# PixelClear/OclPathTracer

Measured on AMD Instinct MI355X. Metric: Msamples/sec (pixels x spp / s), cornellbox.bin 1024x1024, higher is better.
Workload: dtype f32; 1 GPU; BASELINE configs[2]: cornellbox.bin 1024x1024, 256 spp, depth 16, full path; render_lanes=2, checkpointed_launches=True, staging_ring_bytes=402653184, workspace_bytes=477453648

## Files before the change

### oclpathtracer_amd/csrc/pt_kernels.h

```cpp
#pragma once

#include <hip/hip_runtime.h>
#include <stdint.h>

struct PtRawTriangle { float p1[4], p2[4], p3[4]; int32_t id; char pad[12]; };
struct PtRawMaterial { float albedo[4], emissive[4]; float roughness; int32_t type; char pad[24]; };
static_assert(sizeof(PtRawTriangle) == 64 && sizeof(PtRawMaterial) == 64, "record layout");

struct PtPrepTriangle {
    float p1[3];
    float e1[3];
    float e2[3];
    float pad0[3];
    float n[3];
    int32_t id;
};
static_assert(sizeof(PtPrepTriangle) == 64, "prep layout");

struct PtBvhNode {
    float lmin[3]; uint32_t link_l;
    float lmax[3]; uint32_t link_r;
    float rmin[3]; uint32_t pad0;
    float rmax[3]; uint32_t pad1;
};
// ... 24 lines not shown
#define PT_LDS_TRI_STRIDE 12
#define PT_LDS_TRI_MAX 256

struct PtCamera {
    float eye[3], view[3], hol[3], up[3];
    float angle;
};

struct PtTraceParams {
    const PtPrepTriangle* tris;
    const PtRawMaterial* mats;
    float* rad;
    float* rad1;
    unsigned int* batch_counter;
    unsigned long long* stats;
    int32_t width, height;
    float inv_width, inv_height, aspect;
    int32_t frame_begin;
    int32_t frame_count;
    uint32_t chunk_f0;
    uint32_t slot_frames;
    uint32_t ring_phase;
    uint32_t ring_magic;
    uint32_t rad1_off;
    int32_t max_bounces, ntri, nmat;
    int32_t stripe_rows, n_ranks, rank;
    uint32_t npix_local;
    uint32_t batches_per_frame, total_batches;
    uint32_t batch;
    float quad_delta1;
    float ray_radius;
    const float* p1tab;
    float p1_lo, p1_hi;
    const PtBvh8Node* bvh;
    int32_t bvh_records;
    PtBvhGrid grid;
    const PtPrepTriangle* bigtab;
    const int32_t* bigidx;
    int32_t nbig;
    const uint2* pmask;
    unsigned int* bvh_flags;
    int32_t bvh_stack_limit;
    uint32_t* carry;
    uint32_t carry_in_waves;
    uint32_t carry_out;
    PtCamera cam;
};
#define PT_QUEUE_SHARDS 8
#define PT_QUEUE_SHARD_WORDS 1056
#define PT_QUEUE_STOP_WORD (PT_QUEUE_SHARDS * PT_QUEUE_SHARD_WORDS)
#define PT_QUEUE_WORDS ((PT_QUEUE_SHARDS + 1) * PT_QUEUE_SHARD_WORDS)
#define PT_CARRY_RECORDS 64
#define PT_CARRY_STRIDE_DW (16 + PT_CARRY_RECORDS * 15)

struct PtFoldParams {
    const float* rad;
    float4* fb;
    uint32_t npix_local;
    int32_t frame_begin, frame_count;
    unsigned int* reset_counter;
    unsigned int* reset_counter2;
};

#define PT_PREP_WORDS 12
__host__ __device__ static inline unsigned ptk_order_key(float f)
{
    unsigned u;
    __builtin_memcpy(&u, &f, sizeof u);
    return (u & 0x80000000u) ? ~u : (u | 0x80000000u);
}
__host__ __device__ static inline float ptk_order_float(unsigned k)
{
    const unsigned u = (k & 0x80000000u) ? (k & 0x7fffffffu) : ~k;
    float f;
    __builtin_memcpy(&f, &u, sizeof f);
    return f;
}
hipError_t ptk_prep_triangles(const PtRawTriangle* raw, PtPrepTriangle* out, int ntri, unsigned int* det_bound_bits,
                              hipStream_t s);
hipError_t ptk_prep_quad_margins(PtPrepTriangle* out, int ntri, float diameter, float delta1, float* p1tab, const float anchor[3], hipStream_t s);
#define PT_P1_STRIDE 24
static inline size_t ptk_p1tab_floats(int ntri) { return (size_t)((ntri / 2 + 1) / 2) * PT_P1_STRIDE; }
hipError_t ptk_primary_masks(const PtTraceParams& p, hipStream_t s);
struct PtSearchMode {
    bool bvh;
    bool det_bounded;
    int quads;
};
hipError_t ptk_trace(const PtTraceParams& p, int num_blocks, PtSearchMode m, bool tally, bool wide, hipStream_t s);
#define PT_BVH_NEAR_EYE 4.0f
hipError_t ptk_bvh_big_raw(const PtRawTriangle* raw, const int* bigidx, int nbig, PtRawTriangle* out, hipStream_t s);
static inline size_t ptk_bvh_record_count(int ntri) { return 2 * (size_t)(ntri > 0 ? ntri : 0); }
size_t ptk_bvh_temp_bytes(int ntri);
#define PT_BVH_BIG_MAX 64
#define PT_BVH_RAY_EPS 1.2e-4f
hipError_t ptk_bvh_build(const PtRawTriangle* raw, const PtPrepTriangle* prep, int ntri, PtBvh8Node* recs,
                         PtPrepTriangle* bigtab, int* bigidx, int* nbig_dev, PtBvhGrid* grid_dev, unsigned* used_dev, void* temp, size_t temp_bytes,
                         hipStream_t s);
#define PT_DET_BOUND_MAX 2.0e19f
#define PT_BVH_AUTO_MIN 512
hipError_t ptk_fold(const PtFoldParams& p, hipStream_t s);
hipError_t ptk_assemble_stripes(const float4* gathered, float4* image, int width, int height, int stripe_rows,
                                int n_ranks, int slab_rows, hipStream_t s);
hipError_t ptk_tonemap_ppm(const float4* fb, int32_t* rgb, size_t npix, hipStream_t s);
hipError_t ptk_fill_i32(int32_t* dst, int32_t value, int n, hipStream_t s);
hipError_t ptk_math(const float* in, float* out, int n, hipStream_t s);
// ... 139 lines not shown
```

### oclpathtracer_amd/csrc/pt_kernels.hip

```cpp
#include "pt_kernels.h"

#include "pt_device_math.h"

#include <type_traits>

typedef const __attribute__((address_space(4))) float* pt_const_f32p;

PTK_DEV unsigned pt_lane_id() { return __builtin_amdgcn_mbcnt_hi(~0u, __builtin_amdgcn_mbcnt_lo(~0u, 0u)); }
PTK_DEV unsigned pt_mbcnt(unsigned long long m) { return __builtin_amdgcn_mbcnt_hi((unsigned)(m >> 32), __builtin_amdgcn_mbcnt_lo((unsigned)m, 0u)); }

typedef const __attribute__((address_space(4))) PtTraceParams* pt_kargs_p;
PTK_DEV pt_kargs_p pt_kargs()
{
    pt_kargs_p k = (pt_kargs_p)__builtin_amdgcn_kernarg_segment_ptr();
    asm volatile("" : "+s"(k));
    return k;
}
PTK_DEV f3 pt_anchor()
{
    const pt_kargs_p K = pt_kargs();
    return mk3(K->cam.eye[0], K->cam.eye[1], K->cam.eye[2]);
}
#define PT_ARG(field) (LATE ? K->field : P.field)

// ... 625 lines not shown
            for (int jj = 0; jj < n; ++jj) {
                const PtTriRec r = pt_load_tri(T, base + jj);
                float pvx = pt_fma(d.y, r.e2z, -(d.z * r.e2y));
                float pvy = pt_fma(d.z, r.e2x, -(d.x * r.e2z));
                float pvz = pt_fma(d.x, r.e2y, -(d.y * r.e2x));
                float det = pt_fma(r.e1z, pvz, pt_fma(r.e1y, pvy, r.e1x * pvx));
                bool keep = !(det < 1e-8f || -det > 1e-8f);
                float inv_det = 1.0f / det;
                float tvx = o.x - r.p1x, tvy = o.y - r.p1y, tvz = o.z - r.p1z;
                float u = pt_fma(tvz, pvz, pt_fma(tvy, pvy, tvx * pvx)) * inv_det;
                keep = keep && !(u < 0.0f || u > 1.0f);
                float qvx = pt_fma(tvy, r.e1z, -(tvz * r.e1y));
                float qvy = pt_fma(tvz, r.e1x, -(tvx * r.e1z));
                float qvz = pt_fma(tvx, r.e1y, -(tvy * r.e1x));
                float v = pt_fma(d.z, qvz, pt_fma(d.y, qvy, d.x * qvx)) * inv_det;
                keep = keep && !(v < 0.0f || u + v > 1.0f);
                float tt = pt_fma(r.e2z, qvz, pt_fma(r.e2y, qvy, r.e2x * qvx)) * inv_det;
                keep = keep && (tt > 0.0f && tt < 1e20f);
                mx |= (keep ? 1u : 0u) << (n - 1 - jj);
            }
            atomicAdd(&vstat[0], (unsigned long long)n);
            atomicAdd(&vstat[1], (unsigned long long)__popc(mx));
            atomicAdd(&vstat[2], (unsigned long long)__popc(m));
            atomicAdd(&vstat[3], (unsigned long long)__popc(mx & ~m));
        }
#endif
        if (!alive) m = 0u;
        pt_pass2_chunk<DET_BOUNDED, LDS_TABLE>(m, base, n, tris, o, d, tmax, hu, hv, hidx, tl, lane, steps);
    }
    pt_pass2_finish<DET_BOUNDED, LDS_TABLE>(tris, o, d, tmax, hu, hv, hidx, tl, lane, steps);
    return steps;
}


struct PtPath {
    f3 o, d;
    f3 mask, L;
    uint32_t seed;
    int bounce;
    unsigned ro;
    unsigned fl;
};

PTK_DEV unsigned pt_ring_offset(unsigned lp, unsigned frame)
{
    const pt_kargs_p KR = pt_kargs();
    const unsigned fr = frame + KR->ring_phase, S = KR->slot_frames;
    const unsigned r = fr - __umulhi(fr, KR->ring_magic) * (2u * S);
    const bool upper = r >= S;
    return (upper ? KR->rad1_off : 0u) + ((upper ? r - S : r) * KR->npix_local + lp) * 12u;
}


template <bool DET_BOUNDED, bool LATE>
PTK_DEV bool pt_shade_path(const PtTraceParams& P, PtPath& s, float tmax, float hu, float hv, int hidx)
{
    const pt_kargs_p K = pt_kargs();
    bool finished = false;
    if (hidx < 0) {
        const float bg = pt_max(0.45f, 0.0f);
        s.L = add3(s.L, scale3(s.mask, bg));
        finished = true;
    } else {
        float phi = PTK_TWO_PI * pt_random_float(s.seed);
        float xi = pt_random_float(s.seed);
        float sp, cp;
        __builtin_amdgcn_sched_barrier(0);
        pt_sincos(phi, sp, cp);
        __builtin_amdgcn_sched_barrier(0);

        const float4 nid = *reinterpret_cast<const float4*>(reinterpret_cast<const char*>(PT_ARG(tris)) + (size_t)((unsigned)hidx * 64u) + 48);
        const f3 N = mk3(nid.x, nid.y, nid.z);
        const int nm1 = PT_ARG(nmat) - 1;
        int mid = __float_as_int(nid.w);
        mid = mid < 0 ? 0 : mid;
        mid = mid > nm1 ? nm1 : mid;
        f3 p = add3(s.o, scale3(s.d, tmax));
        float w = 1.0f - hu - hv;
        f3 n = normalize3(add3(add3(scale3(N, hu), scale3(N, hv)), scale3(N, w)));

        const PtRawMaterial* mat = reinterpret_cast<const PtRawMaterial*>(reinterpret_cast<const char*>(PT_ARG(mats)) + (size_t)((unsigned)mid * 64u));
        const float4 alb = *reinterpret_cast<const float4*>(mat->albedo);
        const float4 emi = *reinterpret_cast<const float4*>(mat->emissive);
        const float rough = mat->roughness;
        const int type = mat->type;

        s.L.x = s.L.x + s.mask.x * emi.x * 3.0f;
        s.L.y = s.L.y + s.mask.y * emi.y * 3.0f;
        s.L.z = s.L.z + s.mask.z * emi.z * 3.0f;

        n = dot3(n, s.d) < 0.0f ? n : scale3(n, -1.0f);
        f3 wo = neg3(s.d);

        f3 axis = __builtin_fabsf(n.x) > 0.001f ? mk3(0.0f, 1.0f, 0.0f) : mk3(1.0f, 0.0f, 0.0f);
        f3 tv = normalize3(cross3(axis, n));
        f3 sv = cross3(n, tv);
        float cos_arg = 1.0f - xi;
#if PT_GGX_FAST
        if (type == 2) cos_arg = pt_div_by(cos_arg, xi * (rough * rough - 1.0f) + 1.0f);
#else
        if (type == 2) cos_arg = cos_arg / (xi * (rough * rough - 1.0f) + 1.0f);
#endif
        const float cosTheta = pt_sqrt(cos_arg);
        const float sin_arg = type == 2 ? pt_max(0.0f, 1.0f - cosTheta * cosTheta) : xi;
        const float sinTheta = pt_sqrt(sin_arg);
        f3 a = scale3(scale3(sv, cp), sinTheta);
        f3 b = scale3(scale3(tv, sp), sinTheta);
        f3 c = scale3(n, cosTheta);
        f3 sdir = normalize3_unit(add3(add3(a, b), c));

        f3 wi = sdir;
        f3 color = mk3(0.0f, 0.0f, 0.0f);
        float pdf = 0.0f;
        float dwin = 0.0f;
        if (type == 1) {
            dwin = dot3(wi, n);
            pdf = dwin * PTK_INV_PI;
            color = mk3(alb.x * PTK_INV_PI, alb.y * PTK_INV_PI, alb.z * PTK_INV_PI);
        } else if (type == 2) {
            float k2 = 2.0f * dot3(wo, sdir);
            wi = add3(neg3(wo), scale3(sdir, k2));
            dwin = dot3(wi, n);
            float dwon = dot3(wo, n);
            if (!(dwin * dwon < 0.0f)) {
                float r2 = rough * rough;
                const float gd = cosTheta * cosTheta * (r2 - 1.0f) + 1.0f;
#if PT_GGX_FAST
                const float D = pt_div(r2 * PTK_INV_PI, gd * gd);
                float g;
                pt_div_pair(D * cosTheta, 4.0f * dot3(wo, sdir), D, 4.0f * dwin * dwon, pdf, g);
#else
                float D = r2 * PTK_INV_PI / (gd * gd);
                pdf = D * cosTheta / (4.0f * dot3(wo, sdir));
                float g = D / (4.0f * dwin * dwon);
#endif
                color = mk3(alb.x * g * 2.0f, alb.y * g * 2.0f, alb.z * g * 2.0f);
            }
        }
        if (pdf <= 0.0f) {
            finished = true;
        } else {
            float qx = color.x * dwin, qy = color.y * dwin, qz = color.z * dwin;
            pt_div3(qx, qy, qz, pdf);
            s.mask.x = s.mask.x * qx;
            s.mask.y = s.mask.y * qy;
            s.mask.z = s.mask.z * qz;
            s.bounce++;
            if (s.bounce >= PT_ARG(max_bounces)) {
                finished = true;
            } else {
                s.o = add3(p, scale3(wi, 0.01f));
                s.d = normalize3_unit(wi);
            }
        }
    }
    if (finished) {
        const pt_kargs_p KR = pt_kargs();
        float* const rad = KR->rad;
        const unsigned rad1_off = KR->rad1_off;
        typedef float pt_f3v __attribute__((ext_vector_type(3), aligned(4)));
        pt_f3v v;
        v.x = pt_max(s.L.x, 0.0f);
        v.y = pt_max(s.L.y, 0.0f);
        v.z = pt_max(s.L.z, 0.0f);
        if (rad1_off != 0u) {
            *reinterpret_cast<pt_f3v*>(reinterpret_cast<char*>(rad) + (size_t)s.ro) = v;
        } else {
            const unsigned fr = s.fl + KR->ring_phase, S = KR->slot_frames;
            const unsigned r = fr - __umulhi(fr, KR->ring_magic) * (2u * S);
            float* out = (r < S ? rad : KR->rad1) + ((size_t)(r < S ? r : r - S) * KR->npix_local + s.ro) * 3u;
            *reinterpret_cast<pt_f3v*>(out) = v;
        }
    }
    return finished;
}

template <bool DET_BOUNDED, bool LATE>
PTK_DEV void pt_shade(const PtTraceParams& P, PtPath& s, bool& alive, float tmax, float hu, float hv, int hidx)
{
    if (pt_shade_path<DET_BOUNDED, LATE>(P, s, tmax, hu, hv, hidx)) alive = false;
}

PTK_DEV void pt_flush_counters(const PtTraceParams& P, unsigned lane, unsigned n_rays, unsigned n_samples)
{
    if (!P.stats) return;
    const unsigned long long r = n_rays, s = n_samples;
    if (lane == 0) {
        atomicAdd(&P.stats[0], s);
        atomicAdd(&P.stats[1], r);
    }
}

#define PT_POOL 64

struct PtWaveQueue {
    unsigned pix, end, frame;
    unsigned row, col;
    unsigned sl, within;
    unsigned g;
};

#define PT_Q_EMPTY 0xffffffffu

template <bool LATE>
PTK_DEV void pt_queue_locate(const PtTraceParams& P, pt_kargs_p K, PtWaveQueue& q)
{
    q.row = q.pix / (unsigned)PT_ARG(width);
    q.col = q.pix - q.row * (unsigned)PT_ARG(width);
    q.sl = q.row / (unsigned)PT_ARG(stripe_rows);
    q.within = q.row - q.sl * (unsigned)PT_ARG(stripe_rows);
}

template <bool LATE>
PTK_DEV bool pt_queue_refill(const PtTraceParams& P, unsigned lane, PtWaveQueue& q, unsigned empty_mask)
{
    const pt_kargs_p K = pt_kargs();
    if (q.pix != q.end) return true;
    if (q.g == PT_Q_EMPTY) return false;
    const unsigned total = PT_ARG(total_batches);
    unsigned sh = q.g, b = 0u;
    bool got = false;
    for (unsigned tries = 0u; tries < PT_QUEUE_SHARDS && total != 0u; ++tries, sh = (sh + 1u) & (PT_QUEUE_SHARDS - 1u)) {
        if ((empty_mask >> sh) & 1u) continue;
        unsigned k = 0u;
        if (lane == 0) k = atomicAdd(PT_ARG(batch_counter) + sh * PT_QUEUE_SHARD_WORDS, 1u);
        k = __builtin_amdgcn_readfirstlane(k);
        b = k * PT_QUEUE_SHARDS + sh;
        if (b < total) { got = true; break; }
        unsigned seen = 0u;
        if (lane == 0u) seen = atomicOr(PT_ARG(batch_counter) + PT_QUEUE_STOP_WORD, 1u << sh);
        empty_mask |= (1u << sh) | (unsigned)__builtin_amdgcn_readfirstlane(seen);
    }
    if (!got) { q.g = PT_Q_EMPTY; return false; }
    q.g = sh;
    const unsigned f = b / PT_ARG(batches_per_frame);
    const unsigned bi = b - f * PT_ARG(batches_per_frame);
    q.frame = PT_ARG(chunk_f0) + f;
    q.pix = bi * PT_ARG(batch);
    const unsigned e = q.pix + PT_ARG(batch);
    q.end = e < PT_ARG(npix_local) ? e : PT_ARG(npix_local);
    pt_queue_locate<LATE>(P, K, q);
    return true;
}

struct PtPathSlots {
    float4* A;
    unsigned* W;
    unsigned fs, ws, wk;
    PTK_DEV float4& vec(unsigned j, unsigned k) const { return A[j * fs + k]; }
    PTK_DEV unsigned& word(unsigned j, unsigned k) const { return W[j * ws + wk * k]; }
};

#define PT_POOL_DWORDS (PT_POOL * 15)
PTK_DEV PtPathSlots pt_pool_slots(float4* pool) { return { pool, reinterpret_cast<unsigned*>(pool + 3 * PT_POOL), PT_POOL, 1u, 3u }; }
PTK_DEV PtPathSlots pt_carry_slots(uint32_t* region) { return { (float4*)(region + 16), region + 16 + PT_CARRY_RECORDS * 12, PT_CARRY_RECORDS, PT_CARRY_RECORDS, 1u }; }

PTK_DEV void pt_path_store(const PtPathSlots& S, unsigned k, const PtPath& s)
{
    S.vec(0, k) = make_float4(s.o.x, s.o.y, s.o.z, s.d.x);
    S.vec(1, k) = make_float4(s.d.y, s.d.z, s.mask.x, s.mask.y);
    S.vec(2, k) = make_float4(s.mask.z, s.L.x, s.L.y, s.L.z);
    S.word(0, k) = s.seed;
    S.word(1, k) = s.ro;
    S.word(2, k) = s.fl | ((unsigned)s.bounce << 16);
}

PTK_DEV void pt_path_load(const PtPathSlots& S, unsigned k, PtPath& s)
{
    const float4 a0 = S.vec(0, k), a1 = S.vec(1, k), a2 = S.vec(2, k);
    const unsigned w2 = S.word(2, k);
    s.o = mk3(a0.x, a0.y, a0.z);
    s.d = mk3(a0.w, a1.x, a1.y);
    s.mask = mk3(a1.z, a1.w, a2.x);
    s.L = mk3(a2.y, a2.z, a2.w);
    s.seed = S.word(0, k);
    s.ro = S.word(1, k);
    s.fl = w2 & 0xffffu;
    s.bounce = (int)(w2 >> 16);
}

PTK_DEV void pt_pool_push(float4* pool, unsigned& pool_n, const PtPath& s, pt_lanes& alive)
{
    const pt_lanes live = alive;
    if (PT_ON(live)) {
        const unsigned k = pool_n + pt_mbcnt(live);
        pt_path_store(pt_pool_slots(pool), k, s);
    }
    pool_n += (unsigned)__popcll(live);
    alive = 0ull;
}

PTK_DEV void pt_pool_pop(float4* pool, unsigned& pool_n, PtPath& s, pt_lanes& alive)
{
    const pt_lanes need = ~alive;
    const unsigned n_need = (unsigned)__popcll(need);
    const unsigned take = n_need < pool_n ? n_need : pool_n;
    if (take == 0u) return;
    __builtin_amdgcn_fence(__ATOMIC_RELEASE, "wavefront");
    __builtin_amdgcn_wave_barrier();
    __builtin_amdgcn_fence(__ATOMIC_ACQUIRE, "wavefront");
    const unsigned rank = pt_mbcnt(need);
    const pt_lanes taking = need & PT_LANES(rank < take);
    if (PT_ON(taking)) {
        const unsigned k = pool_n - 1u - rank;
        pt_path_load(pt_pool_slots(pool), k, s);
    }
    alive |= taking;
    pool_n -= take;
    __builtin_amdgcn_fence(__ATOMIC_RELEASE, "wavefront");
    __builtin_amdgcn_wave_barrier();
    __builtin_amdgcn_fence(__ATOMIC_ACQUIRE, "wavefront");
}


PTK_DEV void pt_carry_header(uint32_t* region, unsigned n, const PtWaveQueue& q, unsigned n_rays, unsigned n_samples, unsigned n_carried)
{
    region[0] = n;
    region[1] = q.pix;
    region[2] = q.end;
    region[3] = q.frame;
    region[4] = n_rays;
    region[5] = n_samples;
    region[6] = n_carried + n + (q.end - q.pix);
}

PTK_DEV void pt_carry_store(uint32_t* region, unsigned lane, float4* pool, unsigned pool_n, const PtWaveQueue& q, unsigned n_rays, unsigned n_samples,
                            unsigned n_carried)
{
    __builtin_amdgcn_fence(__ATOMIC_RELEASE, "wavefront");
    __builtin_amdgcn_wave_barrier();
    __builtin_amdgcn_fence(__ATOMIC_ACQUIRE, "wavefront");
    if (lane < pool_n) {
        const PtPathSlots from = pt_pool_slots(pool), to = pt_carry_slots(region);
        for (unsigned j = 0; j < 3u; ++j) to.vec(j, lane) = from.vec(j, lane);
        for (unsigned j = 0; j < 3u; ++j) to.word(j, lane) = from.word(j, lane);
    }
    if (lane == 0u) pt_carry_header(region, pool_n, q, n_rays, n_samples, n_carried);
}

PTK_DEV void pt_carry_store_lanes(uint32_t* region, unsigned lane, const PtPath& s, bool alive, const PtWaveQueue& q, unsigned n_rays, unsigned n_samples,
                                  unsigned n_carried)
{
    const unsigned long long live = __ballot(alive);
    const unsigned n_live = (unsigned)__popcll(live);
    if (alive) {
        const unsigned k = pt_mbcnt(live);
        pt_path_store(pt_carry_slots(region), k, s);
    }
    if (lane == 0u) pt_carry_header(region, n_live, q, n_rays, n_samples, n_carried);
}

template <bool LATE>
PTK_DEV void pt_carry_load(const PtTraceParams& P, uint32_t* region, unsigned lane, PtPath& s, bool& alive, PtWaveQueue& q, unsigned& n_rays,
                           unsigned& n_samples, unsigned& n_carried)
{
    const pt_kargs_p K = pt_kargs();
    const unsigned n = __builtin_amdgcn_readfirstlane(region[0]);
    n_rays = __builtin_amdgcn_readfirstlane(region[4]);
    n_samples = __builtin_amdgcn_readfirstlane(region[5]);
    n_carried = __builtin_amdgcn_readfirstlane(region[6]);
    q.pix = __builtin_amdgcn_readfirstlane(region[1]);
    q.end = __builtin_amdgcn_readfirstlane(region[2]);
    q.frame = __builtin_amdgcn_readfirstlane(region[3]);
    pt_queue_locate<LATE>(P, K, q);
    if (lane < n) {
        pt_path_load(pt_carry_slots(region), lane, s);
        alive = true;
    }
}

template <bool LATE>
PTK_DEV int pt_queue_next(const PtTraceParams& P, unsigned lane, PtWaveQueue& q, const PtPath& s, pt_lanes alive)
{
    const pt_kargs_p K = pt_kargs();
    unsigned empty_mask = 0u;
    if (PT_ARG(carry_out) != 0u) {
        if (lane == 0u) empty_mask = __hip_atomic_load(PT_ARG(batch_counter) + PT_QUEUE_STOP_WORD, __ATOMIC_RELAXED, __HIP_MEMORY_SCOPE_AGENT);
        empty_mask = (unsigned)__builtin_amdgcn_readfirstlane(empty_mask);
        if (empty_mask == (1u << PT_QUEUE_SHARDS) - 1u && !(q.pix != q.end && q.frame < PT_ARG(chunk_f0)) && (alive & PT_LANES(s.fl < PT_ARG(chunk_f0))) == 0ull)
            return 2;
    }
    return pt_queue_refill<LATE>(P, lane, q, empty_mask) ? 1 : 0;
}

template <bool LATE>
PTK_DEV unsigned pt_stripe_row(const PtTraceParams& P, pt_kargs_p K, unsigned sl, unsigned within)
{
    return (sl * (unsigned)PT_ARG(n_ranks) + (unsigned)PT_ARG(rank)) * (unsigned)PT_ARG(stripe_rows) + within;
}

template <bool LATE>
PTK_DEV void pt_pixel_xy(const PtTraceParams& P, pt_kargs_p K, unsigned lp, unsigned& x, unsigned& grow)
{
    const unsigned lr = lp / (unsigned)PT_ARG(width);
    x = lp - lr * (unsigned)PT_ARG(width);
    grow = lr;
    if (PT_ARG(n_ranks) > 1) {
        const unsigned sl = lr / (unsigned)PT_ARG(stripe_rows);
        grow = pt_stripe_row<LATE>(P, K, sl, lr - sl * (unsigned)PT_ARG(stripe_rows));
    }
}

template <bool LATE>
PTK_DEV void pt_sample_begin(const PtTraceParams& P, pt_kargs_p K, unsigned x, unsigned grow, unsigned lp, unsigned frame, PtPath& s)
{
    const unsigned gid = grow * (unsigned)PT_ARG(width) + x;
    const int f = PT_ARG(frame_begin) - (int)PT_ARG(chunk_f0) + (int)frame;
    s.seed = gid + pt_hash_u32((uint32_t)f);
    pt_generate_ray((int)x, (int)grow, PT_ARG(inv_width), PT_ARG(inv_height), PT_ARG(aspect), PT_CAM_K(K->cam), s.seed, s.o, s.d);
    s.mask = mk3(1.0f, 1.0f, 1.0f);
    s.L = mk3(0.0f, 0.0f, 0.0f);
    s.bounce = 0;
    s.ro = K->rad1_off != 0u ? pt_ring_offset(lp, frame) : lp;
    s.fl = frame;
}

template <bool LATE>
PTK_DEV bool pt_start_fresh(const PtTraceParams& P, unsigned lane, PtWaveQueue& q, PtPath& s, pt_lanes& alive, unsigned& pix0)
{
    const pt_kargs_p K = pt_kargs();
    pix0 = q.pix;
    const unsigned avail = q.end - q.pix;
    const unsigned count = avail < 64u ? avail : 64u;
    const unsigned W = (unsigned)PT_ARG(width), SR = (unsigned)PT_ARG(stripe_rows);
    if (lane < count) {
        unsigned x = q.col + lane, up = 0u;
        while (x >= W) { x -= W; ++up; }
        unsigned grow = q.row + up;
        if (PT_ARG(n_ranks) > 1) {
            unsigned sl = q.sl, within = q.within + up;
            while (within >= SR) { within -= SR; ++sl; }
            grow = pt_stripe_row<LATE>(P, K, sl, within);
        }
        pt_sample_begin<LATE>(P, K, x, grow, q.pix + lane, q.frame, s);
    }
    alive = count == 64u ? ~0ull : (1ull << count) - 1ull;
    q.pix += count;
    q.col += count;
    while (q.col >= W) {
        q.col -= W;
        ++q.row;
        if (++q.within == SR) { q.within = 0u; ++q.sl; }
    }
    return count == 64u;
}

PTK_DEV PtPath pt_path_idle()
{
    PtPath s;
    s.o = mk3(0.0f, 0.0f, 0.0f); s.d = mk3(0.0f, 0.0f, 1.0f);
    s.mask = mk3(1.0f, 1.0f, 1.0f); s.L = mk3(0.0f, 0.0f, 0.0f);
    s.seed = 0; s.bounce = 0; s.ro = 0; s.fl = 0;
    return s;
}

PTK_DEV unsigned pt_wave_in_wg() { return (unsigned)__builtin_amdgcn_readfirstlane(threadIdx.x >> 6); }
PTK_DEV unsigned pt_wave() { return blockIdx.x * (PT_TRACE_THREADS / 64) + pt_wave_in_wg(); }
PTK_DEV uint32_t* pt_carry_region(uint32_t* carry, unsigned wave) { return carry + (size_t)wave * PT_CARRY_STRIDE_DW; }

PTK_DEV PtTail pt_tail_init(pt_lds_u32* w, unsigned tile, unsigned lane)
{
    PtTail tl;
    tl.keys = (pt_lds_u64*)w;
    tl.list = w + 128;
    tl.wr = tl.rd = 0u;
    tl.kbest = ~0ull; tl.ku = tl.kv = 0.0f;
    tl.tile = tile;
    tl.keys[lane] = ~0ull;
    return tl;
}

PTK_DEV void pt_lds_table_load(const PtPrepTriangle* tris, int n)
{
    const float* g = reinterpret_cast<const float*>(tris);
    for (int k = (int)threadIdx.x; k < n * PT_LDS_TRI_STRIDE; k += PT_TRACE_THREADS) {
        const int tri = k / PT_LDS_TRI_STRIDE, w = k - tri * PT_LDS_TRI_STRIDE;
        pt_lds_tab[k] = g[tri * 16 + w];
    }
}

#define PT_LDS_TILE_DW (32u * PT_LDS_TRI_STRIDE)
template <int LDS_TABLE> __host__ __device__ __forceinline__ unsigned pt_lds_tail_dw() { return 128u + (LDS_TABLE == 1 ? PT_TAIL_LIST / 2u : PT_TAIL_LIST); }
template <int LDS_TABLE> __host__ __device__ __forceinline__ unsigned pt_lds_pools(int ntri) { return LDS_TABLE == 1 ? ntri * PT_LDS_TRI_STRIDE : 0; }
template <int LDS_TABLE, bool POOLS = true> __host__ __device__ __forceinline__ unsigned pt_lds_tails(int ntri) { return pt_lds_pools<LDS_TABLE>(ntri) + (POOLS ? (PT_TRACE_THREADS / 64) * PT_POOL_DWORDS : 0u); }
template <int LDS_TABLE, bool POOLS = true> __host__ __device__ __forceinline__ unsigned pt_lds_tiles(int ntri) { return pt_lds_tails<LDS_TABLE, POOLS>(ntri) + (PT_TRACE_THREADS / 64) * pt_lds_tail_dw<LDS_TABLE>(); }
template <int LDS_TABLE, bool POOLS = true> __host__ __device__ __forceinline__ unsigned pt_lds_total(int ntri) { return pt_lds_tiles<LDS_TABLE, POOLS>(ntri) + (LDS_TABLE == 2 ? (PT_TRACE_THREADS / 64) * PT_LDS_TILE_DW : 0u); }

#ifndef PT_TRACE_UNIT_DIR
#define PT_TRACE_UNIT_DIR 1
#endif
template <bool DET_BOUNDED, int LDS_TABLE, int QUADS>
PTK_DEV void pt_trace_body(const PtTraceParams& P)
{
    const unsigned lane = pt_lane_id();
    pt_const_f32p T = (pt_const_f32p)(const float*)P.tris;
    const int ntri = P.ntri;
    if (LDS_TABLE == 1) {
        pt_lds_table_load(P.tris, ntri);
        __syncthreads();
    }
    const unsigned wave_in_wg = pt_wave_in_wg();
    float4* pool = reinterpret_cast<float4*>(pt_lds_tab + pt_lds_pools<LDS_TABLE>(ntri) + wave_in_wg * PT_POOL_DWORDS);
    unsigned pool_n = 0u;
    PtTail tl = pt_tail_init((pt_lds_u32*)pt_lds_tab + pt_lds_tails<LDS_TABLE>(ntri) + (threadIdx.x >> 6) * pt_lds_tail_dw<LDS_TABLE>(),
                             pt_lds_tiles<LDS_TABLE>(ntri) + (threadIdx.x >> 6) * PT_LDS_TILE_DW, lane);

    PtWaveQueue q = { 0u, 0u, 0u, 0u, 0u, 0u, 0u, 0u };
    pt_lanes alive = 0ull;
    PtPath s = pt_path_idle();
    unsigned n_rays = 0, n_samples = 0, n_carried = 0;
    const unsigned wave = pt_wave();
    if (wave < P.carry_in_waves) {
        bool resumed = false;
        pt_carry_load<true>(P, pt_carry_region(P.carry, wave), lane, s, resumed, q, n_rays, n_samples, n_carried);
        alive = PT_LANES(resumed);
    }
    q.g = wave & (PT_QUEUE_SHARDS - 1u);
#if PT_STAMPS
    unsigned long long t0 = 0, t1 = 0, t2 = 0, t3 = 0, c_regen = 0, c_loop = 0, c_shade = 0, c_iters = 0, c_steps = 0, c_p1 = 0;
#endif

    for (;;) {
        PT_STAMP(t0);
        bool primary = false;
        unsigned pix0 = 0u;
        if (~alive != 0ull) {
            if (pool_n == 0u) {
                const int next = pt_queue_next<true>(P, lane, q, s, alive);
                if (next != 0) {
                    pt_pool_push(pool, pool_n, s, alive);
                    if (next == 2) break;
                    primary = pt_start_fresh<true>(P, lane, q, s, alive, pix0);
                }
            }
            pt_pool_pop(pool, pool_n, s, alive);
        }
        if (alive == 0ull) break;
        PT_STAMP(t1);

        float tmax = 1e20f, hu = 0.0f, hv = 0.0f;
        int hidx = -1;
        unsigned p2steps = 0;
        if (QUADS == 3 && DET_BOUNDED && primary && P.pmask != nullptr)
            p2steps = pt_intersect_primary<DET_BOUNDED, LDS_TABLE>(T, P.tris, ntri, s.o, s.d, PT_ON(alive), tmax, hu, hv, hidx, P.pmask[pix0 + lane], tl, lane,
                                                                   PT_VALIDATE_FILTER && P.stats ? P.stats + 2 : nullptr);
        else
            p2steps = pt_intersect_two_pass<DET_BOUNDED, LDS_TABLE, QUADS, PT_TRACE_UNIT_DIR != 0>(T, P.tris, ntri, s.o, s.d, PT_ON(alive), tmax, hu, hv, hidx,
                                                                                          P.quad_delta1, P.ray_radius,
                                                                                          (pt_const_f32p)P.p1tab, P.p1_lo, P.p1_hi, pt_anchor(), tl, lane,
                                                                                          PT_VALIDATE_FILTER && P.stats ? P.stats + 2 : nullptr,
#if PT_STAMPS
                                                                                          &c_p1
#else
                                                                                          nullptr
#endif
                                                                                          );
#if PT_STAMPS
        c_steps += p2steps;
#else
        (void)p2steps;
#endif

        PT_STAMP(t2);
        n_rays += (unsigned)__popcll(alive);
        bool finished = false;
        if (PT_ON(alive)) finished = pt_shade_path<DET_BOUNDED, true>(P, s, tmax, hu, hv, hidx);
        const pt_lanes done = PT_LANES(finished);
        n_samples += (unsigned)__popcll(done);
        alive &= ~done;
#if PT_STAMPS
        PT_STAMP(t3);
        c_regen += t1 - t0; c_loop += t2 - t1; c_shade += t3 - t2; c_iters++;
#endif
    }

#if PT_STAMPS
    if (P.stats && lane == 0) {
        atomicAdd(&P.stats[2], c_regen);
        atomicAdd(&P.stats[3], c_loop);
        atomicAdd(&P.stats[4], c_shade);
        atomicAdd(&P.stats[5], c_iters);
        atomicAdd(&P.stats[7], c_steps);
        atomicAdd(&P.stats[6], c_p1);
    }
#endif
    {
        const pt_kargs_p K = pt_kargs();
        if (K->carry_out != 0u) {
            pt_carry_store(pt_carry_region(K->carry, wave), lane, pool, pool_n, q, n_rays, n_samples, n_carried);
            return;
        }
    }
#if !PT_STAMPS && !PT_VALIDATE_FILTER
    if (P.stats && lane == 0 && n_carried != 0u) atomicAdd(&P.stats[7], (unsigned long long)n_carried);
#endif
    pt_flush_counters(P, lane, n_rays, n_samples);
}

#ifndef PT_TRACE_WAVES
#define PT_TRACE_WAVES 8
#endif
template <bool DET_BOUNDED, int LDS_TABLE, int QUADS>
__global__ __launch_bounds__(PT_TRACE_THREADS) __attribute__((amdgpu_waves_per_eu(PT_TRACE_WAVES, PT_TRACE_WAVES)))
void pt_trace_kernel(const PtTraceParams P)
{
    pt_trace_body<DET_BOUNDED, LDS_TABLE, QUADS>(P);
}

template <bool DET_BOUNDED>
__global__ __launch_bounds__(PT_TRACE_THREADS) __attribute__((amdgpu_waves_per_eu(6, 6)))
void pt_trace_tiled_kernel(const PtTraceParams P)
{
    pt_trace_body<DET_BOUNDED, 2, 0>(P);
}

#ifndef PT_BVH_STACK
#define PT_BVH_STACK 64
#endif
#ifndef PT_BVH_LDS_STACK
#define PT_BVH_LDS_STACK 8
#endif
#ifndef PT_BVH_REFILL
#define PT_BVH_REFILL 40
#endif

#define PT_BVH_TAIL_DW (128u + PT_TAIL_LIST)
__host__ __device__ __forceinline__ unsigned pt_bvh_lds_stacks() { return PT_BVH_BIG_MAX * PT_LDS_TRI_STRIDE; }
__host__ __device__ __forceinline__ unsigned pt_bvh_lds_tails() { return pt_bvh_lds_stacks() + 2 * PT_BVH_LDS_STACK * PT_TRACE_THREADS; }
__host__ __device__ __forceinline__ unsigned pt_bvh_lds_nxt() { return pt_bvh_lds_tails() + (PT_TRACE_THREADS / 64) * PT_BVH_TAIL_DW; }
__host__ __device__ __forceinline__ unsigned pt_bvh_lds_total() { return pt_bvh_lds_nxt() + 2048u / 4u; }

template <bool LATE>
PTK_DEV void pt_regenerate_lanes(const PtTraceParams& P, unsigned lane, PtWaveQueue& q, PtPath& s, bool& alive)
{
    const pt_kargs_p K = pt_kargs();
    unsigned long long need = __ballot(!alive);
    while (need != 0ull && pt_queue_refill<true>(P, lane, q, 0u)) {
        const unsigned n_need = (unsigned)__popcll(need);
        const unsigned avail = q.end - q.pix;
        const unsigned take = n_need < avail ? n_need : avail;
        const unsigned rank = pt_mbcnt(need);
        if (!alive && rank < take) {
// ... 2785 lines not shown
```

### oclpathtracer_amd/csrc/pt_shim.hip

```cpp
#include "../../include/pt_shim.h"

#include <hip/hip_runtime.h>

#include <algorithm>
#include <cmath>
#include <cstdarg>
#include <cstdio>
#include <cstdlib>
#include <cstring>
#include <initializer_list>
#include <new>
#include <string>
#include <utility>
#include <vector>

#include "pt_kernels.h"

static thread_local char g_err[512] = "";

static int fail(int code, const char* fmt, ...)
{
    va_list ap;
    va_start(ap, fmt);
    vsnprintf(g_err, sizeof g_err, fmt, ap);
// ... 1174 lines not shown
static int choose_batch(const pt_device_s* d, bool use_bvh, uint32_t npix, int chunk, uint32_t& batch, uint32_t& bpf, int& blocks)
{
    const int wg_waves = PT_TRACE_THREADS / 64;
    blocks = d->prop.multiProcessorCount * (use_bvh ? d->bvh_blocks_per_cu : d->blocks_per_cu);
    const uint64_t resident_waves = (uint64_t)blocks * wg_waves;
    const uint64_t chunk_samples = (uint64_t)npix * (uint64_t)chunk;
    batch = PT_TRACE_BATCH;
    while (batch > 128u && chunk_samples / batch < 64u * resident_waves) batch >>= 1;
    bpf = (npix + batch - 1) / batch;
    if ((uint64_t)bpf * (uint64_t)chunk + PT_QUEUE_SHARDS > 0xffffffffull) return fail(PT_ERR_INVALID, "chunk too large");
    const uint64_t blocks_needed = ((uint64_t)bpf * (uint64_t)chunk + wg_waves - 1) / wg_waves;
    if ((uint64_t)blocks > blocks_needed) blocks = (int)blocks_needed;
    return PT_OK;
}

static void image_geometry(PtTraceParams& t, int width, int height, int stripe_rows, int n_ranks, int rank, uint32_t npix)
{
    t.width = width; t.height = height;
    t.inv_width = 1.0f / (float)width;
    t.inv_height = 1.0f / (float)height;
    t.aspect = (float)width / (float)height;
    t.stripe_rows = stripe_rows; t.n_ranks = n_ranks; t.rank = rank;
    t.npix_local = npix;
}

static PtTraceParams trace_params(const pt_device_s* d, const pt_buffer_s* mats, const pt_buffer_s* stats, const pt_render_params& rp,
                                  const PtCamera& cam, uint32_t npix, const PtSearch& search, bool use_pmask, int chunk, uint32_t batch, uint32_t bpf)
{
    PtTraceParams tp;
    memset(&tp, 0, sizeof tp);
    search_fields(d, search, tp);
    tp.mats = (const PtRawMaterial*)mats->dptr;
    tp.stats = stats ? (unsigned long long*)stats->dptr : nullptr;
    image_geometry(tp, rp.width, rp.height, rp.stripe_rows, rp.n_ranks, rp.rank, npix);
    tp.max_bounces = rp.max_bounces; tp.nmat = rp.num_materials;
    tp.batches_per_frame = bpf; tp.batch = batch;
    tp.pmask = use_pmask ? d->pmask.p : nullptr;
    tp.slot_frames = (uint32_t)chunk;
    tp.ring_magic = (uint32_t)(0x100000000ull / (2u * (uint32_t)chunk)) + 1u;
    tp.rad = d->ring;
    tp.rad1 = reinterpret_cast<float*>(reinterpret_cast<char*>(d->ring.p) + d->ring_slot_bytes);
    tp.rad1_off = (uint64_t)PT_RING_SLOTS * d->ring_slot_bytes <= 0x100000000ull ? (uint32_t)d->ring_slot_bytes : 0u;
    tp.cam = cam;
    return tp;
}

static int ensure_carry(pt_device_s* d, int blocks)
{
    const int wg_waves = PT_TRACE_THREADS / 64;
    const size_t waves = (size_t)d->prop.multiProcessorCount * 8 * wg_waves;
    if ((size_t)blocks * wg_waves > waves) return fail(PT_ERR_INVALID, "grid larger than the checkpoint regions");
    for (int k = 0; k < 2; ++k)
        if (!d->carry[k]) {
            hipError_t e = ws_malloc(d, d->carry[k], waves * PT_CARRY_STRIDE_DW * sizeof(uint32_t));
            if (e != hipSuccess) return fail(PT_ERR_OOM, "checkpoint buffer allocation failed: %s", hipGetErrorString(e));
        }
    return PT_OK;
}

static int render_part(pt_device_s* d, pt_buffer_s* tris, pt_buffer_s* mats, pt_buffer_s* fb, const pt_render_params& rp, const PtCamera& cam,
                       uint32_t npix, pt_buffer_s* stats, pt_event_s* ev_start, pt_event_s* ev_stop)
{
    int rc;
    PtSearch search;
    if ((rc = prepare_search(d, tris, rp.num_triangles, cam.eye, search))) return rc;
    const bool use_bvh = search.mode.bvh;
    int nchunks, chunk;
    if ((rc = plan_chunks(d, rp.frame_count, npix, nchunks, chunk))) return rc;
    const bool want_pmask = d->opt_pmask && search.mode.quads == 3 && !use_bvh && rp.num_triangles <= 64 && search.mode.det_bounded;
    const bool use_pmask = want_pmask && pmask_footprint_holds(rp.width, rp.height);
    if (want_pmask && !use_pmask) d->pmask_key.valid = false;
    bool make_pmask = false;
    if (use_pmask && (rc = refresh_pmask(d, rp, cam, npix, make_pmask))) return rc;
    if (d->counters_dirty) {
        if ((rc = stream_enqueue(d))) return rc;
        HIP_TRY(hipMemsetAsync(d->counters, 0, WS_COUNTERS, d->stream));
        d->counters_dirty = false;
    }
    uint32_t batch, bpf;
    int blocks;
    if ((rc = choose_batch(d, use_bvh, npix, chunk, batch, bpf, blocks))) return rc;
    PtTraceParams tp = trace_params(d, mats, stats, rp, cam, npix, search, use_pmask, chunk, batch, bpf);
    if (make_pmask) {
        HIP_TRY(ptk_primary_masks(tp, d->stream));
        d->pmask_key.valid = true;
    }
    const bool carry = d->opt_carry != 0 && nchunks > 1;
    int ln = d->opt_lanes == 2 ? (int)(d->render_seq++ & 1u) : 0;
    hipStream_t st = d->lane[ln];
    if (carry && (rc = ensure_carry(d, blocks))) return rc;
    const int wg_waves = PT_TRACE_THREADS / 64;

    if (d->main_dirty || d->external) {
        HIP_TRY(hipEventRecord(d->ev_fork, d->stream));
        HIP_TRY(hipStreamWaitEvent(d->lane[0], d->ev_fork, 0));
        HIP_TRY(hipStreamWaitEvent(d->lane[1], d->ev_fork, 0));
        d->main_dirty = false;
    }
    d->lanes_busy = true;
    d->counters_dirty = true;
    if (ev_start) HIP_TRY(hipEventRecord(ev_start->start, st));
    tp.ring_phase = (uint32_t)((d->chunk_seq & 1u) ? chunk : 0);
    tp.carry = carry ? d->carry[ln].p : nullptr;
    unsigned int* const drain_counter = d->counters + (size_t)(PT_QUEUE_COUNTERS - 1 - ln) * PT_QUEUE_STRIDE;
    unsigned int* prev_counter = nullptr;
    int prev_slot = 0, prev_f0 = 0, prev_nf = 0;
    hipEvent_t pstop;
    bool chained = false;
    auto fold = [&](int slot, int f0, int nf, unsigned int* reset, unsigned int* reset2) -> int {
        const bool last = f0 + nf >= rp.frame_count || !carry, last_two = f0 + nf + chunk >= rp.frame_count;
        if ((!chained || !carry) && d->fold_recorded[ln ^ 1]) HIP_TRY(hipStreamWaitEvent(st, d->ev_fold[ln ^ 1], 0));
        chained = true;
        PtFoldParams fp;
        fp.rad = slot ? tp.rad1 : tp.rad;
        fp.fb = (float4*)fb->dptr;
        fp.npix_local = npix;
        fp.frame_begin = rp.frame_begin + f0;
        fp.frame_count = nf;
        fp.reset_counter = reset;
// ... 1135 lines not shown
```

Baseline: 9271 Msamples/s.

## Defer shading to the next loop iteration and park hit records in the pool

Reorders the persistent trace loop so a lane's intersection result (hit point, barycentrics, triangle index) is stored with the path and shaded at the top of the next iteration, after pool refill. Paths parked in the LDS pool or the checkpoint regions now carry their pending hit, so shading runs on a compacted wave instead of one thinned out by finished lanes. Pool records grow by a float4 plus a packed word, so the pool shrinks from 64 to 56 entries to fit LDS, and the checkpoint stride grows. Bounce count and triangle index are packed in 8 bits each, which adds a new max_bounces limit for small non-BVH scenes.

```diff
diff --git a/oclpathtracer_amd/csrc/pt_kernels.h b/oclpathtracer_amd/csrc/pt_kernels.h
--- a/oclpathtracer_amd/csrc/pt_kernels.h
+++ b/oclpathtracer_amd/csrc/pt_kernels.h
@@ -100,6 +100,8 @@
 #define PT_QUEUE_WORDS ((PT_QUEUE_SHARDS + 1) * PT_QUEUE_SHARD_WORDS)
 #define PT_CARRY_RECORDS 64
 #define PT_CARRY_STRIDE_DW (16 + PT_CARRY_RECORDS * 15)
+#define PT_CARRY_HIT_STRIDE_DW (16 + PT_CARRY_RECORDS * 18)
+#define PT_PACKED_BOUNCE_MAX 256
 
 struct PtFoldParams {
     const float* rad;
diff --git a/oclpathtracer_amd/csrc/pt_kernels.hip b/oclpathtracer_amd/csrc/pt_kernels.hip
--- a/oclpathtracer_amd/csrc/pt_kernels.hip
+++ b/oclpathtracer_amd/csrc/pt_kernels.hip
@@ -701,16 +701,19 @@
 }
 
 
+
+PTK_DEV void pt_shade_miss(PtPath& s)
+{
+    const float bg = pt_max(0.45f, 0.0f);
+    s.L = add3(s.L, scale3(s.mask, bg));
+}
+
 template <bool DET_BOUNDED, bool LATE>
-PTK_DEV bool pt_shade_path(const PtTraceParams& P, PtPath& s, float tmax, float hu, float hv, int hidx)
+PTK_DEV bool pt_shade_hit(const PtTraceParams& P, PtPath& s, const f3 p, float hu, float hv, int hidx)
 {
     const pt_kargs_p K = pt_kargs();
     bool finished = false;
-    if (hidx < 0) {
-        const float bg = pt_max(0.45f, 0.0f);
-        s.L = add3(s.L, scale3(s.mask, bg));
-        finished = true;
-    } else {
+    {
         float phi = PTK_TWO_PI * pt_random_float(s.seed);
         float xi = pt_random_float(s.seed);
         float sp, cp;
@@ -724,7 +727,6 @@
         int mid = __float_as_int(nid.w);
         mid = mid < 0 ? 0 : mid;
         mid = mid > nm1 ? nm1 : mid;
-        f3 p = add3(s.o, scale3(s.d, tmax));
         float w = 1.0f - hu - hv;
         f3 n = normalize3(add3(add3(scale3(N, hu), scale3(N, hv)), scale3(N, w)));
 
@@ -803,7 +805,12 @@
             }
         }
     }
-    if (finished) {
+    return finished;
+}
+
+PTK_DEV void pt_path_finish(const PtPath& s)
+{
+    {
         const pt_kargs_p KR = pt_kargs();
         float* const rad = KR->rad;
         const unsigned rad1_off = KR->rad1_off;
@@ -821,6 +828,19 @@
             *reinterpret_cast<pt_f3v*>(out) = v;
         }
     }
+}
+
+template <bool DET_BOUNDED, bool LATE>
+PTK_DEV bool pt_shade_path(const PtTraceParams& P, PtPath& s, float tmax, float hu, float hv, int hidx)
+{
+    bool finished = false;
+    if (hidx < 0) {
+        pt_shade_miss(s);
+        finished = true;
+    } else {
+        finished = pt_shade_hit<DET_BOUNDED, LATE>(P, s, add3(s.o, scale3(s.d, tmax)), hu, hv, hidx);
+    }
+    if (finished) pt_path_finish(s);
     return finished;
 }
 
@@ -840,7 +860,7 @@
     }
 }
 
-#define PT_POOL 64
+#define PT_POOL 56
 
 struct PtWaveQueue {
     unsigned pix, end, frame;
@@ -900,9 +920,59 @@
     PTK_DEV unsigned& word(unsigned j, unsigned k) const { return W[j * ws + wk * k]; }
 };
 
-#define PT_POOL_DWORDS (PT_POOL * 15)
-PTK_DEV PtPathSlots pt_pool_slots(float4* pool) { return { pool, reinterpret_cast<unsigned*>(pool + 3 * PT_POOL), PT_POOL, 1u, 3u }; }
 PTK_DEV PtPathSlots pt_carry_slots(uint32_t* region) { return { (float4*)(region + 16), region + 16 + PT_CARRY_RECORDS * 12, PT_CARRY_RECORDS, PT_CARRY_RECORDS, 1u }; }
+
+static_assert(PT_LDS_TRI_MAX <= 256 && PT_PACKED_BOUNCE_MAX <= 256, "triangle and bounce count of a parked path: 8 bits each of the packed word");
+template <int LDS_TABLE> __host__ __device__ constexpr unsigned pt_hit_words() { return LDS_TABLE == 1 ? 1u : 2u; }
+template <int LDS_TABLE> __host__ __device__ constexpr unsigned pt_pool_dwords() { return PT_POOL * (16u + pt_hit_words<LDS_TABLE>()); }
+static_assert(pt_pool_dwords<1>() % 4u == 0u && pt_pool_dwords<2>() % 4u == 0u, "a wave's pool must be a whole number of float4: the next pool's 16-byte alignment");
+static_assert(PT_POOL <= PT_CARRY_RECORDS, "a checkpoint region holds a whole pool");
+template <unsigned NW> PTK_DEV PtPathSlots pt_pool_slots(float4* pool) { return { pool, reinterpret_cast<unsigned*>(pool + 4 * PT_POOL), PT_POOL, 1u, NW }; }
+PTK_DEV PtPathSlots pt_carry_hit_slots(uint32_t* region) { return { (float4*)(region + 16), region + 16 + PT_CARRY_RECORDS * 16, PT_CARRY_RECORDS, PT_CARRY_RECORDS, 1u }; }
+
+struct PtHit {
+    float hu, hv;
+    int hidx;
+};
+
+template <unsigned NW>
+PTK_DEV void pt_hit_store(const PtPathSlots& S, unsigned k, const PtPath& s, const PtHit& h)
+{
+    S.vec(0, k) = make_float4(s.o.x, s.o.y, s.o.z, s.d.x);
+    S.vec(1, k) = make_float4(s.d.y, s.d.z, s.mask.x, s.mask.y);
+    S.vec(2, k) = make_float4(s.mask.z, s.L.x, s.L.y, s.L.z);
+    S.vec(3, k) = make_float4(__uint_as_float(s.seed), __uint_as_float(s.ro), h.hu, h.hv);
+    const unsigned w = s.fl | ((unsigned)s.bounce << 16);
+    if (NW == 1u) {
+        S.word(0, k) = w | ((unsigned)h.hidx << 24);
+    } else {
+        S.word(0, k) = w;
+        S.word(1, k) = (unsigned)h.hidx;
+    }
+}
+
+template <unsigned NW>
+PTK_DEV void pt_hit_load(const PtPathSlots& S, unsigned k, PtPath& s, PtHit& h)
+{
+    const float4 a0 = S.vec(0, k), a1 = S.vec(1, k), a2 = S.vec(2, k), a3 = S.vec(3, k);
+    const unsigned w = S.word(0, k);
+    s.o = mk3(a0.x, a0.y, a0.z);
+    s.d = mk3(a0.w, a1.x, a1.y);
+    s.mask = mk3(a1.z, a1.w, a2.x);
+    s.L = mk3(a2.y, a2.z, a2.w);
+    s.seed = __float_as_uint(a3.x);
+    s.ro = __float_as_uint(a3.y);
+    h.hu = a3.z;
+    h.hv = a3.w;
+    s.fl = w & 0xffffu;
+    if (NW == 1u) {
+        s.bounce = (int)((w >> 16) & 0xffu);
+        h.hidx = (int)(w >> 24);
+    } else {
+        s.bounce = (int)(w >> 16);
+        h.hidx = (int)S.word(1, k);
+    }
+}
 
 PTK_DEV void pt_path_store(const PtPathSlots& S, unsigned k, const PtPath& s)
 {
@@ -928,18 +998,20 @@
     s.bounce = (int)(w2 >> 16);
 }
 
-PTK_DEV void pt_pool_push(float4* pool, unsigned& pool_n, const PtPath& s, pt_lanes& alive)
+template <unsigned NW>
+PTK_DEV void pt_pool_push(float4* pool, unsigned& pool_n, const PtPath& s, const PtHit& h, pt_lanes& alive)
 {
     const pt_lanes live = alive;
     if (PT_ON(live)) {
         const unsigned k = pool_n + pt_mbcnt(live);
-        pt_path_store(pt_pool_slots(pool), k, s);
+        pt_hit_store<NW>(pt_pool_slots<NW>(pool), k, s, h);
     }
     pool_n += (unsigned)__popcll(live);
     alive = 0ull;
 }
 
-PTK_DEV void pt_pool_pop(float4* pool, unsigned& pool_n, PtPath& s, pt_lanes& alive)
+template <unsigned NW>
+PTK_DEV void pt_pool_pop(float4* pool, unsigned& pool_n, PtPath& s, PtHit& h, pt_lanes& alive)
 {
     const pt_lanes need = ~alive;
     const unsigned n_need = (unsigned)__popcll(need);
@@ -952,7 +1024,7 @@
     const pt_lanes taking = need & PT_LANES(rank < take);
     if (PT_ON(taking)) {
         const unsigned k = pool_n - 1u - rank;
-        pt_path_load(pt_pool_slots(pool), k, s);
+        pt_hit_load<NW>(pt_pool_slots<NW>(pool), k, s, h);
     }
     alive |= taking;
     pool_n -= take;
@@ -973,6 +1045,7 @@
     region[6] = n_carried + n + (q.end - q.pix);
 }
 
+template <unsigned NW>
 PTK_DEV void pt_carry_store(uint32_t* region, unsigned lane, float4* pool, unsigned pool_n, const PtWaveQueue& q, unsigned n_rays, unsigned n_samples,
                             unsigned n_carried)
 {
@@ -980,9 +1053,9 @@
     __builtin_amdgcn_wave_barrier();
     __builtin_amdgcn_fence(__ATOMIC_ACQUIRE, "wavefront");
     if (lane < pool_n) {
-        const PtPathSlots from = pt_pool_slots(pool), to = pt_carry_slots(region);
-        for (unsigned j = 0; j < 3u; ++j) to.vec(j, lane) = from.vec(j, lane);
-        for (unsigned j = 0; j < 3u; ++j) to.word(j, lane) = from.word(j, lane);
+        const PtPathSlots from = pt_pool_slots<NW>(pool), to = pt_carry_hit_slots(region);
+        for (unsigned j = 0; j < 4u; ++j) to.vec(j, lane) = from.vec(j, lane);
+        for (unsigned j = 0; j < NW; ++j) to.word(j, lane) = from.word(j, lane);
     }
     if (lane == 0u) pt_carry_header(region, pool_n, q, n_rays, n_samples, n_carried);
 }
@@ -1000,8 +1073,7 @@
 }
 
 template <bool LATE>
-PTK_DEV void pt_carry_load(const PtTraceParams& P, uint32_t* region, unsigned lane, PtPath& s, bool& alive, PtWaveQueue& q, unsigned& n_rays,
-                           unsigned& n_samples, unsigned& n_carried)
+PTK_DEV unsigned pt_carry_header_load(const PtTraceParams& P, const uint32_t* region, PtWaveQueue& q, unsigned& n_rays, unsigned& n_samples, unsigned& n_carried)
 {
     const pt_kargs_p K = pt_kargs();
     const unsigned n = __builtin_amdgcn_readfirstlane(region[0]);
@@ -1012,8 +1084,27 @@
     q.end = __builtin_amdgcn_readfirstlane(region[2]);
     q.frame = __builtin_amdgcn_readfirstlane(region[3]);
     pt_queue_locate<LATE>(P, K, q);
+    return n;
+}
+
+template <bool LATE>
+PTK_DEV void pt_carry_load(const PtTraceParams& P, uint32_t* region, unsigned lane, PtPath& s, bool& alive, PtWaveQueue& q, unsigned& n_rays,
+                           unsigned& n_samples, unsigned& n_carried)
+{
+    const unsigned n = pt_carry_header_load<LATE>(P, region, q, n_rays, n_samples, n_carried);
     if (lane < n) {
         pt_path_load(pt_carry_slots(region), lane, s);
+        alive = true;
+    }
+}
+
+template <bool LATE, unsigned NW>
+PTK_DEV void pt_carry_hit_load(const PtTraceParams& P, uint32_t* region, unsigned lane, PtPath& s, PtHit& h, bool& alive, PtWaveQueue& q, unsigned& n_rays,
+                               unsigned& n_samples, unsigned& n_carried)
+{
+    const unsigned n = pt_carry_header_load<LATE>(P, region, q, n_rays, n_samples, n_carried);
+    if (lane < n) {
+        pt_hit_load<NW>(pt_carry_hit_slots(region), lane, s, h);
         alive = true;
     }
 }
@@ -1105,7 +1196,7 @@
 
 PTK_DEV unsigned pt_wave_in_wg() { return (unsigned)__builtin_amdgcn_readfirstlane(threadIdx.x >> 6); }
 PTK_DEV unsigned pt_wave() { return blockIdx.x * (PT_TRACE_THREADS / 64) + pt_wave_in_wg(); }
-PTK_DEV uint32_t* pt_carry_region(uint32_t* carry, unsigned wave) { return carry + (size_t)wave * PT_CARRY_STRIDE_DW; }
+PTK_DEV uint32_t* pt_carry_region(uint32_t* carry, unsigned wave, unsigned stride = PT_CARRY_STRIDE_DW) { return carry + (size_t)wave * stride; }
 
 PTK_DEV PtTail pt_tail_init(pt_lds_u32* w, unsigned tile, unsigned lane)
 {
@@ -1131,7 +1222,7 @@
 #define PT_LDS_TILE_DW (32u * PT_LDS_TRI_STRIDE)
 template <int LDS_TABLE> __host__ __device__ __forceinline__ unsigned pt_lds_tail_dw() { return 128u + (LDS_TABLE == 1 ? PT_TAIL_LIST / 2u : PT_TAIL_LIST); }
 template <int LDS_TABLE> __host__ __device__ __forceinline__ unsigned pt_lds_pools(int ntri) { return LDS_TABLE == 1 ? ntri * PT_LDS_TRI_STRIDE : 0; }
-template <int LDS_TABLE, bool POOLS = true> __host__ __device__ __forceinline__ unsigned pt_lds_tails(int ntri) { return pt_lds_pools<LDS_TABLE>(ntri) + (POOLS ? (PT_TRACE_THREADS / 64) * PT_POOL_DWORDS : 0u); }
+template <int LDS_TABLE, bool POOLS = true> __host__ __device__ __forceinline__ unsigned pt_lds_tails(int ntri) { return pt_lds_pools<LDS_TABLE>(ntri) + (POOLS ? (PT_TRACE_THREADS / 64) * pt_pool_dwords<LDS_TABLE>() : 0u); }
 template <int LDS_TABLE, bool POOLS = true> __host__ __device__ __forceinline__ unsigned pt_lds_tiles(int ntri) { return pt_lds_tails<LDS_TABLE, POOLS>(ntri) + (PT_TRACE_THREADS / 64) * pt_lds_tail_dw<LDS_TABLE>(); }
 template <int LDS_TABLE, bool POOLS = true> __host__ __device__ __forceinline__ unsigned pt_lds_total(int ntri) { return pt_lds_tiles<LDS_TABLE, POOLS>(ntri) + (LDS_TABLE == 2 ? (PT_TRACE_THREADS / 64) * PT_LDS_TILE_DW : 0u); }
 
@@ -1149,7 +1240,8 @@
         __syncthreads();
     }
     const unsigned wave_in_wg = pt_wave_in_wg();
-    float4* pool = reinterpret_cast<float4*>(pt_lds_tab + pt_lds_pools<LDS_TABLE>(ntri) + wave_in_wg * PT_POOL_DWORDS);
+    constexpr unsigned NW = pt_hit_words<LDS_TABLE>();
+    float4* pool = reinterpret_cast<float4*>(pt_lds_tab + pt_lds_pools<LDS_TABLE>(ntri) + wave_in_wg * pt_pool_dwords<LDS_TABLE>());
     unsigned pool_n = 0u;
     PtTail tl = pt_tail_init((pt_lds_u32*)pt_lds_tab + pt_lds_tails<LDS_TABLE>(ntri) + (threadIdx.x >> 6) * pt_lds_tail_dw<LDS_TABLE>(),
                              pt_lds_tiles<LDS_TABLE>(ntri) + (threadIdx.x >> 6) * PT_LDS_TILE_DW, lane);
@@ -1157,11 +1249,13 @@
     PtWaveQueue q = { 0u, 0u, 0u, 0u, 0u, 0u, 0u, 0u };
     pt_lanes alive = 0ull;
     PtPath s = pt_path_idle();
+    PtHit h = { 0.0f, 0.0f, -1 };
+    pt_lanes ended = 0ull;
     unsigned n_rays = 0, n_samples = 0, n_carried = 0;
     const unsigned wave = pt_wave();
     if (wave < P.carry_in_waves) {
         bool resumed = false;
-        pt_carry_load<true>(P, pt_carry_region(P.carry, wave), lane, s, resumed, q, n_rays, n_samples, n_carried);
+        pt_carry_hit_load<true, NW>(P, pt_carry_region(P.carry, wave, PT_CARRY_HIT_STRIDE_DW), lane, s, h, resumed, q, n_rays, n_samples, n_carried);
         alive = PT_LANES(resumed);
     }
     q.g = wave & (PT_QUEUE_SHARDS - 1u);
@@ -1171,26 +1265,47 @@
 
     for (;;) {
         PT_STAMP(t0);
+        {
+            const pt_lanes missed = alive & PT_LANES(h.hidx < 0);
+            if (PT_ON(missed)) pt_shade_miss(s);
+            const pt_lanes over = missed | ended;
+            if (PT_ON(over)) pt_path_finish(s);
+            n_samples += (unsigned)__popcll(over);
+            alive &= ~missed;
+            ended = 0ull;
+        }
+        bool fresh = false;
         bool primary = false;
         unsigned pix0 = 0u;
         if (~alive != 0ull) {
-            if (pool_n == 0u) {
+            if (pool_n == 0u && (unsigned)__popcll(alive) <= (unsigned)PT_POOL) {
                 const int next = pt_queue_next<true>(P, lane, q, s, alive);
                 if (next != 0) {
-                    pt_pool_push(pool, pool_n, s, alive);
+                    pt_pool_push<NW>(pool, pool_n, s, h, alive);
                     if (next == 2) break;
                     primary = pt_start_fresh<true>(P, lane, q, s, alive, pix0);
+                    fresh = true;
                 }
             }
-            pt_pool_pop(pool, pool_n, s, alive);
-        }
-        if (alive == 0ull) break;
+            if (!fresh) pt_pool_pop<NW>(pool, pool_n, s, h, alive);
+        }
+        if (!fresh && alive == 0ull) break;
         PT_STAMP(t1);
+
+        if (!fresh) {
+            bool finished = false;
+            if (PT_ON(alive)) finished = pt_shade_hit<DET_BOUNDED, true>(P, s, s.o, h.hu, h.hv, h.hidx);
+            ended = PT_LANES(finished);
+            alive &= ~ended;
+        }
+        PT_STAMP(t2);
 
         float tmax = 1e20f, hu = 0.0f, hv = 0.0f;
         int hidx = -1;
         unsigned p2steps = 0;
-        if (QUADS == 3 && DET_BOUNDED && primary && P.pmask != nullptr)
+        n_rays += (unsigned)__popcll(alive);
+        if (alive == 0ull) {
+        } else if (QUADS == 3 && DET_BOUNDED && primary && P.pmask != nullptr)
             p2steps = pt_intersect_primary<DET_BOUNDED, LDS_TABLE>(T, P.tris, ntri, s.o, s.d, PT_ON(alive), tmax, hu, hv, hidx, P.pmask[pix0 + lane], tl, lane,
                                                                    PT_VALIDATE_FILTER && P.stats ? P.stats + 2 : nullptr);
         else
@@ -1210,16 +1325,11 @@
         (void)p2steps;
 #endif
 
-        PT_STAMP(t2);
-        n_rays += (unsigned)__popcll(alive);
-        bool finished = false;
-        if (PT_ON(alive)) finished = pt_shade_path<DET_BOUNDED, true>(P, s, tmax, hu, hv, hidx);
-        const pt_lanes done = PT_LANES(finished);
-        n_samples += (unsigned)__popcll(done);
-        alive &= ~done;
+        s.o = add3(s.o, scale3(s.d, tmax));
+        h.hu = hu; h.hv = hv; h.hidx = hidx;
 #if PT_STAMPS
         PT_STAMP(t3);
-        c_regen += t1 - t0; c_loop += t2 - t1; c_shade += t3 - t2; c_iters++;
+        c_regen += t1 - t0; c_shade += t2 - t1; c_loop += t3 - t2; c_iters++;
 #endif
     }
 
@@ -1236,7 +1346,7 @@
     {
         const pt_kargs_p K = pt_kargs();
         if (K->carry_out != 0u) {
-            pt_carry_store(pt_carry_region(K->carry, wave), lane, pool, pool_n, q, n_rays, n_samples, n_carried);
+            pt_carry_store<NW>(pt_carry_region(K->carry, wave, PT_CARRY_HIT_STRIDE_DW), lane, pool, pool_n, q, n_rays, n_samples, n_carried);
             return;
         }
     }
diff --git a/oclpathtracer_amd/csrc/pt_shim.hip b/oclpathtracer_amd/csrc/pt_shim.hip
--- a/oclpathtracer_amd/csrc/pt_shim.hip
+++ b/oclpathtracer_amd/csrc/pt_shim.hip
@@ -1250,7 +1250,8 @@
     if ((size_t)blocks * wg_waves > waves) return fail(PT_ERR_INVALID, "grid larger than the checkpoint regions");
     for (int k = 0; k < 2; ++k)
         if (!d->carry[k]) {
-            hipError_t e = ws_malloc(d, d->carry[k], waves * PT_CARRY_STRIDE_DW * sizeof(uint32_t));
+            static_assert(PT_CARRY_HIT_STRIDE_DW >= PT_CARRY_STRIDE_DW, "a checkpoint region holds either kernel's records");
+            hipError_t e = ws_malloc(d, d->carry[k], waves * PT_CARRY_HIT_STRIDE_DW * sizeof(uint32_t));
             if (e != hipSuccess) return fail(PT_ERR_OOM, "checkpoint buffer allocation failed: %s", hipGetErrorString(e));
         }
     return PT_OK;
@@ -1263,6 +1264,9 @@
     PtSearch search;
     if ((rc = prepare_search(d, tris, rp.num_triangles, cam.eye, search))) return rc;
     const bool use_bvh = search.mode.bvh;
+    if (!use_bvh && rp.num_triangles <= PT_LDS_TRI_MAX && rp.max_bounces > PT_PACKED_BOUNCE_MAX)
+        return fail(PT_ERR_INVALID, "max_bounces above %d on a scene of at most %d triangles without the LBVH (a parked path packs its bounce count in 8 bits)",
+                    PT_PACKED_BOUNCE_MAX, PT_LDS_TRI_MAX);
     int nchunks, chunk;
     if ((rc = plan_chunks(d, rp.frame_count, npix, nchunks, chunk))) return rc;
     const bool want_pmask = d->opt_pmask && search.mode.quads == 3 && !use_bvh && rp.num_triangles <= 64 && search.mode.det_bounded;
```

After: 9381 Msamples/s (median of 6 runs). 1.2% higher.
